# feiyeha/EGM-Unet

Measured on AMD Instinct MI355X. Metric: train images/sec at 3x512x512 bs=8/GPU, higher is better.
Workload: dtype bf16; 1 GPU; EGM-UNet GRFBUNet(3,2,base_c=32) fwd+5-term-loss+bwd+SGD, 8x3x512x512 per GPU (BASELINE.json configs[1]); global_batch=8, parallelism=dp1, launch=hipGraph replay, world_size=1

## Files before the change

### egm_unet_amd/csrc/common.h

```cpp
#pragma once
#include <hip/hip_runtime.h>
#include <stdint.h>
#include <stdio.h>
#include <stdlib.h>
#include <string.h>
#include <type_traits>
#include "../../include/egm_hip.h"

void egm_set_error(const char* fmt, ...);
#define EGM_FAIL(code, ...) do { egm_set_error(__VA_ARGS__); return (code); } while (0)
#define EGM_REQUIRE(cond, ...) do { if (!(cond)) EGM_FAIL(EGM_ERR_ARG, __VA_ARGS__); } while (0)
#define EGM_CHECK_LAUNCH(name) do { hipError_t e_ = hipGetLastError(); \
    if (e_ != hipSuccess) EGM_FAIL(EGM_ERR_LAUNCH, "%s: launch failed: %s", name, hipGetErrorString(e_)); } while (0)

static inline bool egm_aligned16(const void* p) { return (reinterpret_cast<uintptr_t>(p) & 15) == 0; }
static inline int egm_cdiv(long long a, long long b) { return (int)((a + b - 1) / b); }
static inline int egm_env_int(const char* name, int dflt) { const char* v = getenv(name); return v ? atoi(v) : dflt; }

template <auto Kernel> int egm_allow_max_lds(const char* what, int bytes = 160 * 1024) {
    static bool done = false;
    if (!done) {
        hipError_t e = hipFuncSetAttribute(reinterpret_cast<const void*>(Kernel), hipFuncAttributeMaxDynamicSharedMemorySize, bytes);
        if (e != hipSuccess) EGM_FAIL(EGM_ERR_LAUNCH, "%s: hipFuncSetAttribute: %s", what, hipGetErrorString(e));
        done = true;
// ... 28 lines not shown
__device__ __forceinline__ float bf16_to_f32(uint16_t b) { return __uint_as_float(((uint32_t)b) << 16); }
__device__ __forceinline__ uint16_t f32_to_bf16(float f) {
    __bf16 h = (__bf16)f;
    return *reinterpret_cast<uint16_t*>(&h);
}

template <typename T> struct TypeInfo;
template <> struct TypeInfo<float>  { static constexpr int kDtype = EGM_F32;  static constexpr int kVec = 4; };
template <> struct TypeInfo<bf16_t> { static constexpr int kDtype = EGM_BF16; static constexpr int kVec = 8; };

__device__ __forceinline__ float to_f32(float x) { return x; }
__device__ __forceinline__ float to_f32(bf16_t x) { return bf16_to_f32(x.v); }
template <typename T> __device__ __forceinline__ T from_f32(float x);
template <> __device__ __forceinline__ float from_f32<float>(float x) { return x; }
template <> __device__ __forceinline__ bf16_t from_f32<bf16_t>(float x) { bf16_t r; r.v = f32_to_bf16(x); return r; }

__device__ __forceinline__ void load8(const float* p, float (&v)[8]) {
    float4 a = *reinterpret_cast<const float4*>(p), b = *reinterpret_cast<const float4*>(p + 4);
    v[0] = a.x; v[1] = a.y; v[2] = a.z; v[3] = a.w; v[4] = b.x; v[5] = b.y; v[6] = b.z; v[7] = b.w;
}
#ifndef EGM_LOAD_MODE
#define EGM_LOAD_MODE 0
#endif
__device__ __forceinline__ void load8(const bf16_t* p, float (&v)[8]) {
#if EGM_LOAD_MODE == 2
    typedef __attribute__((ext_vector_type(4))) unsigned int u32x4_;
    const u32x4_ t = __builtin_nontemporal_load(reinterpret_cast<const u32x4_*>(p));
    uint4 a; a.x = t.x; a.y = t.y; a.z = t.z; a.w = t.w;
#else
    uint4 a = *reinterpret_cast<const uint4*>(p);
#endif
    v[0] = __uint_as_float(a.x << 16); v[1] = __uint_as_float(a.x & 0xffff0000u);
    v[2] = __uint_as_float(a.y << 16); v[3] = __uint_as_float(a.y & 0xffff0000u);
    v[4] = __uint_as_float(a.z << 16); v[5] = __uint_as_float(a.z & 0xffff0000u);
    v[6] = __uint_as_float(a.w << 16); v[7] = __uint_as_float(a.w & 0xffff0000u);
}
#ifndef EGM_STORE_MODE
#define EGM_STORE_MODE 2
#endif
#ifndef EGM_CONV_STORE_MODE
#define EGM_CONV_STORE_MODE 1
#endif
typedef __attribute__((ext_vector_type(4))) unsigned int egm_u32x4;
template <int MODE, typename V>
__device__ __forceinline__ void egm_store16_as(void* p, V a) {
    if (MODE == 1) asm volatile("global_store_dwordx4 %0, %1, off sc1\n\ts_nop 1" :: "v"(p), "v"(a) : "memory");
    else if (MODE == 2) __builtin_nontemporal_store(a, reinterpret_cast<V*>(p));
    else *reinterpret_cast<V*>(p) = a;
}
__device__ __forceinline__ void egm_store16_conv(void* p, uint4 v) {
    egm_u32x4 a; a.x = v.x; a.y = v.y; a.z = v.z; a.w = v.w;
    egm_store16_as<EGM_CONV_STORE_MODE>(p, a);
}
__device__ __forceinline__ void store8(float* p, const float (&v)[8]) {
    *reinterpret_cast<float4*>(p) = make_float4(v[0], v[1], v[2], v[3]);
    *reinterpret_cast<float4*>(p + 4) = make_float4(v[4], v[5], v[6], v[7]);
}
__device__ __forceinline__ void store8(bf16_t* p, const float (&v)[8]) {
// ... 122 lines not shown
```

### egm_unet_amd/csrc/pool_up.hip

```cpp
#include "common.h"

namespace {

template <typename T>
__global__ void nchw_to_nhwc_kernel(const float* __restrict__ src, T* __restrict__ dst, int ld, int N, int C, long long HW) {
    const long long total = (long long)N * HW;
    for (long long i = blockIdx.x * 256LL + threadIdx.x; i < total; i += (long long)gridDim.x * 256) {
        const long long n = i / HW, p = i - n * HW;
        for (int c0 = 0; c0 < ld; c0 += 8) {
            float v[8];
#pragma unroll
            for (int j = 0; j < 8; ++j) v[j] = (c0 + j < C) ? src[(n * C + c0 + j) * HW + p] : 0.f;
            store8(dst + i * ld + c0, v);
        }
    }
}
template <typename T>
__global__ void nhwc_to_nchw_kernel(const T* __restrict__ src, int ld, float* __restrict__ dst, int N, int C, long long HW) {
    const long long total = (long long)N * HW;
    for (long long i = blockIdx.x * 256LL + threadIdx.x; i < total; i += (long long)gridDim.x * 256) {
        const long long n = i / HW, p = i - n * HW;
        for (int c0 = 0; c0 < C; c0 += 8) {
            float v[8];
            load8(src + i * ld + c0, v);
// ... 56 lines not shown
                load8(add + off[k] * ldadd + cv * 8, a);
#pragma unroll
                for (int j = 0; j < 8; ++j) o[k][j] += a[j];
            }
        }
        store8(dx + base * lddx + cv * 8, o[0]);
        store8(dx + (base + 1) * lddx + cv * 8, o[1]);
        store8(dx + (base + W) * lddx + cv * 8, o[2]);
        store8(dx + (base + W + 1) * lddx + cv * 8, o[3]);
    }
}
template <typename T>
__global__ void zero_tail_kernel(T* __restrict__ dx, int lddx, int N, int H, int W, int C) {
    const int ncv = C >> 3;
    const long long total = (long long)N * H * W * ncv;
    float z[8]; zero8(z);
    for (long long i = blockIdx.x * 256LL + threadIdx.x; i < total; i += (long long)gridDim.x * 256) {
        long long p; int cv; egm_divmod(i, ncv, p, cv);
        int xx, yy; egm_pix_yx(p, H, W, yy, xx);
        if (yy >= (H & ~1) || xx >= (W & ~1)) store8(dx + p * lddx + cv * 8, z);
    }
}

struct Lerp { int i0, i1; float w0, w1; };
__device__ __forceinline__ Lerp lerp_coord(int dst, int in_size, int out_size) {
    const float scale = out_size > 1 ? (float)(in_size - 1) / (float)(out_size - 1) : 0.f;
    const float src = scale * (float)dst;
    Lerp l;
    l.i0 = (int)src;
    l.i1 = l.i0 + (l.i0 < in_size - 1 ? 1 : 0);
    l.w1 = src - (float)l.i0;
    l.w0 = 1.f - l.w1;
    return l;
}

template <typename T>
__global__ void upcat_fwd_kernel(const T* __restrict__ skip, int lds, const T* __restrict__ low, int ldl, T* __restrict__ out,
                                 int ldo, int N, int Hs, int Ws, int Cs, int Hl, int Wl, int Cl) {
    const int ncs = Cs >> 3, ncv = (Cs + Cl) >> 3, first = skip ? 0 : ncs, nw = ncv - first;
    const int Hu = 2 * Hl, Wu = 2 * Wl, py = (Hs - Hu) / 2, px = (Ws - Wu) / 2;
    const long long total = (long long)N * Hs * Ws * nw;
    for (long long i = blockIdx.x * 256LL + threadIdx.x; i < total; i += (long long)gridDim.x * 256) {
        const int cv = first + (int)(i % nw); const long long p = i / nw;
        float v[8];
        if (cv < ncs) {
            load8(skip + p * lds + cv * 8, v);
        } else {
            int x, y, n; egm_pix_nyx(p, Hs, Ws, n, y, x);
            const int uy = y - py, ux = x - px, c = (cv - ncs) * 8;
            zero8(v);
            if (uy >= 0 && uy < Hu && ux >= 0 && ux < Wu) {
                const Lerp ly = lerp_coord(uy, Hl, Hu), lx = lerp_coord(ux, Wl, Wu);
                const T* b = low + (long long)n * Hl * Wl * ldl + c;
                float a[8];
                load8(b + ((long long)ly.i0 * Wl + lx.i0) * ldl, a);
#pragma unroll
                for (int j = 0; j < 8; ++j) v[j] += ly.w0 * lx.w0 * a[j];
                load8(b + ((long long)ly.i0 * Wl + lx.i1) * ldl, a);
#pragma unroll
                for (int j = 0; j < 8; ++j) v[j] += ly.w0 * lx.w1 * a[j];
                load8(b + ((long long)ly.i1 * Wl + lx.i0) * ldl, a);
#pragma unroll
                for (int j = 0; j < 8; ++j) v[j] += ly.w1 * lx.w0 * a[j];
                load8(b + ((long long)ly.i1 * Wl + lx.i1) * ldl, a);
#pragma unroll
                for (int j = 0; j < 8; ++j) v[j] += ly.w1 * lx.w1 * a[j];
            }
        }
        store8(out + p * ldo + cv * 8, v);
    }
}

template <typename T>
__global__ void upcat_bwd_low_kernel(const T* __restrict__ dout, int ldo, T* __restrict__ dlow, int ldl, int N, int Hs, int Ws,
                                     int Cs, int Hl, int Wl, int Cl) {
// ... 610 lines not shown
```

### egm_unet_amd/egm_unet.py

```python
import math
from typing import Dict

import torch
import torch.nn as nn

from . import ops
from ._lib import ACT_NONE, ACT_RELU, ACT_SIGMOID
from .unet import DoubleConv, OutConv, Up, _SegNetBase


class StdPool(nn.Module):
    """Holder only (src/EGM-UNet.py:827-834); the statistics come from egm_mca_reduce."""


class MCAGate(nn.Module):
    def __init__(self, k_size, pool_types=("avg", "std")):
        super().__init__()
        self.pools = nn.ModuleList([nn.AdaptiveAvgPool2d(1) if p == "avg" else StdPool() for p in pool_types])
        self.conv = nn.Conv2d(1, 1, kernel_size=(1, k_size), stride=1, padding=(0, (k_size - 1) // 2), bias=False)
        self.sigmoid = nn.Sigmoid()
        self.weight = nn.Parameter(torch.rand(2))
        self.conv._egm_no_prepack = True


# ... 136 lines not shown
            BasicConv(in_channels, i, 3, padding=1),
            BasicConv(i, 2 * i, 3, stride=stride, padding=1, groups=2),
            BasicConv(2 * i, 2 * i, 3, padding=3 * visual, dilation=3 * visual, relu=False),
            BasicConv(2 * i, 2 * i, 1))
        self.concat_channels = in_channels + 6 * i
        self.fusion_conv = FusionConv(self.concat_channels, out_channels, factor=fusion_factor)
        self.shortcut = BasicConv(in_channels, out_channels, 1, stride, relu=False)
        self.relu = nn.ReLU(inplace=False)
        self.target_enhancer = nn.Sequential(nn.Conv2d(out_channels, 3, 3, padding=1), nn.Sigmoid())

    @staticmethod
    def _seq(seq, x, out):
        mods = list(seq)
        for m in mods[:-1]:
            x = m(x)
        return mods[-1](x, out=out)

    def cat_buffer(self, N, H, W, dtype, device):
        C, i2 = self.shortcut.conv.in_channels, 2 * self.inter_planes
        if i2 % 8 or C % 8:
            return None
        return ops.cat_slots(N, H, W, [C, i2, i2, i2], dtype, device)

    def forward(self, x, out=None, cat=None, pool=False):
        edge, x_e2, x_cat, x_sc = ops.fork_highpass3(x, 3)
        xe = self.edge_enhancer(None, x_e2, edge=edge)
        N, H, W, C = x.shape
        if cat is None:
            cat = self.cat_buffer(N, H, W, x.dtype, x.device) if C == self.shortcut.conv.in_channels else None
        if cat is not None:
            buf, (_, sd, se, sc) = cat
        else:
            buf, sd, se, sc = None, None, None, None
        bd, be, bc = self.branch_dir, self.branch_edge, self.branch_ctx
        xe_d, xe_e, xe_c = ops.fork(xe, 3)
        def item(m, t, o=None):
            return (t, m.conv, m.bn, ACT_RELU if m.relu is not None else ACT_NONE, m._dil, m._groups, o)

        d, e, c = ops.multi_conv_bn_act([item(bd[0], xe_d), item(be[0], xe_e), item(bc[0], xe_c)])
        e = be[1](e)
        e, c = ops.multi_conv_bn_act([item(be[2], e), item(bc[1], c)])
        d, e, c = ops.multi_conv_bn_act([item(bd[1], d), item(be[3], e), item(bc[2], c)])
        d, e, c = ops.multi_conv_bn_act([item(bd[2], d, sd), item(be[4], e, se), item(bc[3], c, sc)])
        cat = ops.cat_channels([x_cat, d, e, c], buf)
        out_f = self.fusion_conv(cat)
        sc = self.shortcut
        out_f = ops.conv_bn_ew(x_sc, sc.conv, sc.bn, ACT_NONE, out_f, ops.EW_SAR, alpha=self.scale)
        o_a, o_b = ops.fork(out_f, 2)
# ... 171 lines not shown
    def __init__(self, in_channels, out_channels, mid_channels=None, use_mca=True):
        if mid_channels is None:
            mid_channels = out_channels
        layers = [nn.Conv2d(in_channels, mid_channels, kernel_size=3, padding=1, bias=False), nn.BatchNorm2d(mid_channels), nn.ReLU(inplace=True)]
        if use_mca:
            layers.append(MCALayer(mid_channels))
        layers += [nn.Conv2d(mid_channels, out_channels, kernel_size=3, padding=1, bias=False), nn.BatchNorm2d(out_channels),
                   nn.ReLU(inplace=True), EdgeEnhancedGRFB(mid_channels, out_channels, stride=1, scale=0.1, visual=12)]
        super().__init__(*layers)
        self._mca = use_mca

    def forward(self, x, out=None, pool=False):
        o = 1 if self._mca else 0
        if self._mca:
            if ops.fuse_mca_bn():
                x = self[3](ops.conv_bn_lazy(x, self[0], self[1], ACT_RELU), exclusive=True)
            else:
                x = self[3](ops.conv_bn_act(x, self[0], self[1], ACT_RELU))
        else:
            x = ops.conv_bn_act(x, self[0], self[1], ACT_RELU)
        grfb = self[6 + o]
        N, H, W = x.shape[0], x.shape[1], x.shape[2]
        cat = grfb.cat_buffer(N, H, W, x.dtype, x.device) if self[3 + o].out_channels == grfb.shortcut.conv.in_channels else None
        x = ops.conv_bn_act(x, self[3 + o], self[4 + o], ACT_RELU, out=None if cat is None else cat[1][0])
        return grfb(x, out, cat, pool=pool)


class Down(nn.Sequential):
    def __init__(self, in_channels, out_channels, use_mca=True):
        super().__init__(nn.MaxPool2d(2, stride=2), DoubleConv1(in_channels, out_channels, use_mca=use_mca))

    def forward(self, x, out=None, pooled=None, pool=False):
        return self[1](ops.maxpool2(x) if pooled is None else pooled, out, pool=pool)


class GRFBUNet(_SegNetBase):
    def __init__(self, in_channels: int = 1, num_classes: int = 2, bilinear: bool = True, base_c: int = 64,
                 use_attention: bool = False, use_mca: bool = True):
        super().__init__()
        self.in_channels = in_channels
        self.num_classes = num_classes
        self.bilinear = bilinear
        self.in_conv = DoubleConv(in_channels, base_c)
        self.down1 = Down(base_c, base_c * 2, use_mca)
        self.down2 = Down(base_c * 2, base_c * 4, use_mca)
        self.down3 = Down(base_c * 4, base_c * 8, use_mca)
        factor = 2 if bilinear else 1
# ... 4 lines not shown
        self.up3 = Up(base_c * 4, base_c * 2 // factor, bilinear)
        self.up4 = Up(base_c * 2, base_c, bilinear)
        self.out_conv = OutConv(base_c, num_classes)

    def forward(self, x: torch.Tensor) -> Dict[str, torch.Tensor]:
        x = self._enter(x)
        bufs, slots = [None] * 4, [None] * 4
        if self.bilinear:
            N, H, W, _ = x.shape
            for k, up in enumerate((self.up4, self.up3, self.up2, self.up1)):
                cin = up.conv[0].in_channels
                cs = cin // 2
                h, w = H >> k, W >> k
                if cs % 8 == 0 and cin % 8 == 0 and (h << k) == H and (w << k) == W:
                    bufs[k], (slots[k], _) = ops.cat_slots(N, h, w, [cs, cin - cs], x.dtype, x.device)
        x1s, p1 = self.in_conv(x, slots[0], pool=True)
        x2s, p2 = self.down1(None, slots[1], pooled=p1, pool=True)
        x3s, p3 = self.down2(None, slots[2], pooled=p2, pool=True)
        x4s, p4 = self.down3(None, slots[3], pooled=p3, pool=True)
        d4 = self.down4(None, pooled=p4)
        if self.ddp_boundary is not None:
            self.ddp_boundary.extend([x1s, x2s, x3s, x4s, d4])
        x5 = self.attn1(d4)
        y = self.up1(x5, x4s, bufs[3])
        y = self.up2(y, x3s, bufs[2])
        y = self.up3(y, x2s, bufs[1])
        y = self.up4(y, x1s, bufs[0], lazy="force" if ops.fuse_cls() else False)
        return self._exit(self.out_conv(y, sole_consumer=True))
```

### egm_unet_amd/ops.py

```python
import ctypes
import os
import struct
import threading
import weakref
from collections import namedtuple

import torch
from torch.autograd import Function, Variable

from ._lib import ACT_NONE, ACT_RELU, ACT_SIGMOID, dtype_code, lib, ptr, stream


def pad8(c: int) -> int:
    return (c + 7) // 8 * 8


def _nhwc(t: torch.Tensor):
    assert t.dim() == 4, t.shape
    N, H, W, C = t.shape
    s = t.stride()
    ok = (s[3] == 1 and s[2] % 8 == 0 and s[2] >= C and s[1] == W * s[2] and s[0] == H * W * s[2]
          and t.data_ptr() % 16 == 0 and C % 8 == 0)
    if not ok:
        if C % 8:
# ... 1425 lines not shown
        (x,) = ctx.saved_tensors
        x, ldx = _nhwc(x)
        N, H, W, C = x.shape
        if gy is None:
            return gskip
        gy, ldg = _nhwc(gy)
        gx = torch.empty((N, H, W, C), dtype=x.dtype, device=x.device)
        dt = dtype_code(x.dtype)
        if gskip is None:
            lib().call("egm_maxpool2_bwd", dt, ptr(x), ldx, ptr(gy), ldg, ptr(gx), C, N, H, W, C, stream())
        elif (H | W) & 1:
            lib().call("egm_maxpool2_bwd", dt, ptr(x), ldx, ptr(gy), ldg, ptr(gx), C, N, H, W, C, stream())
            gx = _axpby(gx, 1.0, gskip, 1.0)
        else:
            gs, lds = _nhwc(gskip)
            lib().call("egm_maxpool2_bwd_add", dt, ptr(x), ldx, ptr(gy), ldg, ptr(gs), lds, ptr(gx), C, N, H, W, C, stream())
        return gx


def fork_maxpool2(x):
    return _ForkMaxPool2.apply(x)


class _UpCat(Function):

    @staticmethod
    def forward(ctx, skip, low, catbuf=None):
        skip, lds = _nhwc(skip)
        low, ldl = _nhwc(low)
        N, Hs, Ws, Cs = skip.shape
        _, Hl, Wl, Cl = low.shape
        inplace = False
        if catbuf is not None:
            cb = catbuf[0]
            inplace = (cb.is_contiguous() and tuple(cb.shape) == (N, Hs, Ws, Cs + Cl) and cb.dtype == skip.dtype
                       and cb.data_ptr() == skip.data_ptr() and lds == Cs + Cl)
        if inplace:
            out = cb
            lib().call("egm_upcat_fwd", dtype_code(skip.dtype), None, lds, ptr(low), ldl, ptr(out), Cs + Cl, N, Hs, Ws, Cs,
                       Hl, Wl, Cl, stream())
        else:
            out = torch.empty((N, Hs, Ws, Cs + Cl), dtype=skip.dtype, device=skip.device)
            lib().call("egm_upcat_fwd", dtype_code(skip.dtype), ptr(skip), lds, ptr(low), ldl, ptr(out), Cs + Cl, N, Hs, Ws, Cs,
                       Hl, Wl, Cl, stream())
        ctx.shape = (N, Hs, Ws, Cs, Hl, Wl, Cl)
        return out

    @staticmethod
    def backward(ctx, g):
        N, Hs, Ws, Cs, Hl, Wl, Cl = ctx.shape
        pend = _take_dz(g)
        gskip = glow = None
        if pend is not None:
            _, ga, gb = pend[1]
            if ctx.needs_input_grad[0]:
                gskip = ga
            if ctx.needs_input_grad[1]:
                glow = torch.empty((N, Hl, Wl, Cl), dtype=gb.dtype, device=gb.device)
                lib().call("egm_upcat_bwd_low", dtype_code(gb.dtype), ptr(gb), Cl, ptr(glow), Cl, N, Hs, Ws, 0, Hl, Wl, Cl, stream())
            return gskip, glow, None
        g, ldo = _nhwc(g)
        if ctx.needs_input_grad[0]:
            gskip = g[..., :Cs]
        if ctx.needs_input_grad[1]:
            glow = torch.empty((N, Hl, Wl, Cl), dtype=g.dtype, device=g.device)
            lib().call("egm_upcat_bwd_low", dtype_code(g.dtype), ptr(g), ldo, ptr(glow), Cl, N, Hs, Ws, Cs, Hl, Wl, Cl, stream())
        return gskip, glow, None


def upcat(skip, low, catbuf=None):
    out = _UpCat.apply(skip, low, None if catbuf is None else [catbuf])
    out._egm_split = skip.shape[3]
    return out


class _Fork2(Function):

    @staticmethod
    def forward(ctx, x):
        return x.view_as(x), x.view_as(x)

    @staticmethod
    def backward(ctx, ga, gb):
        if ga is None:
            return gb
        if gb is None:
            return ga
        ga, lda = _nhwc(ga)
        gb, ldb = _nhwc(gb)
        out = torch.empty(ga.shape, dtype=ga.dtype, device=ga.device)
        lib().call("egm_axpby", dtype_code(ga.dtype), ptr(ga), lda, 1.0, ptr(gb), ldb, 1.0, ptr(out), out.shape[3], _npix(ga),
                   ga.shape[3], stream())
        return out

# ... 116 lines not shown

class _Highpass3(Function):
    @staticmethod
    def forward(ctx, x):
        return _hp(x)

    @staticmethod
    def backward(ctx, g):
        return _hp(g)


def highpass3(x):
    return _Highpass3.apply(x)


class _ForkHighpass(Function):

    @staticmethod
    def forward(ctx, x, n):
        return (_hp(x),) + tuple(x.view_as(x) for _ in range(n))

    @staticmethod
    def backward(ctx, ghp, *gs):
        gs = [g for g in gs if g is not None]
        if ghp is None:
            return (_Fork.backward(ctx, *gs)[0] if gs else None), None
        if not gs:
            return _hp(ghp), None
        while len(gs) > 3:
            gs = gs[:2] + [_Fork.backward(ctx, *gs[2:])[0]]
        a, lda = _nhwc(ghp)
        N, H, W, C = a.shape
        ts = [_nhwc(t) for t in gs] + [(None, 0)] * (3 - len(gs))
        out = torch.empty(a.shape, dtype=a.dtype, device=a.device)
        lib().call("egm_sum4_hp", dtype_code(a.dtype), ptr(a), lda, ptr(ts[0][0]), ts[0][1], ptr(ts[1][0]), ts[1][1], ptr(ts[2][0]), ts[2][1],
                   ptr(out), C, N, H, W, C, stream())
        return out, None


def fork_highpass3(x, n):
    return _ForkHighpass.apply(x, n)


class _GateMul(Function):
    @staticmethod
    def forward(ctx, x, w):
        x, ldx = _nhwc(x)
        w, ldw = _nhwc(w)
        out = torch.empty(x.shape, dtype=x.dtype, device=x.device)
        lib().call("egm_gate_mul_fwd", dtype_code(x.dtype), ptr(x), ldx, ptr(w), ldw, ptr(out), x.shape[3], _npix(x), x.shape[3], stream())
        ctx.save_for_backward(x, w)
        return out

    @staticmethod
    def backward(ctx, g):
        x, w = ctx.saved_tensors
        x, ldx = _nhwc(x); w, ldw = _nhwc(w); g, ldg = _nhwc(g)
        C = x.shape[3]
        dx = torch.empty(x.shape, dtype=x.dtype, device=x.device)
        dw = torch.empty(x.shape, dtype=x.dtype, device=x.device)
        lib().call("egm_gate_mul_bwd", dtype_code(x.dtype), ptr(g), ldg, ptr(x), ldx, ptr(w), ldw, ptr(dx), C, ptr(dw), C, _npix(x), C, stream())
        return dx, dw

# ... 747 lines not shown
```

### egm_unet_amd/unet.py

```python
from typing import Dict

import torch
import torch.nn as nn

from . import ops
from ._lib import ACT_RELU, require_gpu


class DoubleConv(nn.Sequential):

    def __init__(self, in_channels, out_channels, mid_channels=None, use_attention=False):
        if mid_channels is None:
            mid_channels = out_channels
        super().__init__(
            nn.Conv2d(in_channels, mid_channels, kernel_size=3, padding=1, bias=False),
            nn.BatchNorm2d(mid_channels),
            nn.ReLU(inplace=True),
            nn.Conv2d(mid_channels, out_channels, kernel_size=3, padding=1, bias=False),
            nn.BatchNorm2d(out_channels),
            nn.ReLU(inplace=True),
        )

    def forward(self, x, out=None, lazy=False, pool=False):
        x = ops.conv_bn_act(x, self[0], self[1], ACT_RELU)
# ... 8 lines not shown

    def __init__(self, in_channels, out_channels):
        super().__init__(nn.MaxPool2d(2, stride=2), DoubleConv(in_channels, out_channels))

    def forward(self, x, pooled=None, pool=False):
        return self[1](ops.maxpool2(x) if pooled is None else pooled, pool=pool)


class Up(nn.Module):

    def __init__(self, in_channels, out_channels, bilinear=True, use_attention=False):
        super().__init__()
        self.bilinear = bilinear
        if bilinear:
            self.up = nn.Upsample(scale_factor=2, mode="bilinear", align_corners=True)
            self.conv = DoubleConv(in_channels, out_channels, in_channels // 2)
        else:
            self.up = nn.ConvTranspose2d(in_channels, in_channels // 2, kernel_size=2, stride=2)
            self.conv = DoubleConv(in_channels, out_channels)

    def forward(self, x1, x2, catbuf=None, lazy=False):
        if self.bilinear:
            return self.conv(ops.upcat(x2, x1, catbuf), lazy=lazy)
        x1 = ops.conv_transpose2x2(x1, self.up, (x2.shape[1], x2.shape[2]))
        return self.conv(ops.cat_channels([x2, x1]), lazy=lazy)


class OutConv(nn.Sequential):

    def __init__(self, in_channels, num_classes):
        super().__init__(nn.Conv2d(in_channels, num_classes, kernel_size=1))

    def forward(self, x, sole_consumer=False):
        if sole_consumer and ops.bn_act_cls_ok(x, self[0].weight):
            out = ops.bn_act_cls(x, self[0].weight, self[0].bias)
            out._egm_nchw_logits = True
            return out
        was_lazy = isinstance(x, ops.Lazy)
        return ops.conv2d(ops.materialize(x), self[0].weight, self[0].bias, defer_dgrad=sole_consumer and not was_lazy)


class _SegNetBase(nn.Module):

    compute_dtype = torch.float32
    ddp_boundary = None

    def set_compute_dtype(self, dtype):
# ... 37 lines not shown
        self.in_conv = DoubleConv(in_channels, base_c)
        self.down1 = Down(base_c, base_c * 2)
        self.down2 = Down(base_c * 2, base_c * 4)
        self.down3 = Down(base_c * 4, base_c * 8)
        factor = 2 if bilinear else 1
        self.down4 = Down(base_c * 8, base_c * 16 // factor)
        self.up1 = Up(base_c * 16, base_c * 8 // factor, bilinear)
        self.up2 = Up(base_c * 8, base_c * 4 // factor, bilinear)
        self.up3 = Up(base_c * 4, base_c * 2 // factor, bilinear)
        self.up4 = Up(base_c * 2, base_c, bilinear)
        self.out_conv = OutConv(base_c, num_classes)

    def forward(self, x: torch.Tensor) -> Dict[str, torch.Tensor]:
        x = self._enter(x)
        x1s, p1 = self.in_conv(x, pool=True)
        x2s, p2 = self.down1(None, pooled=p1, pool=True)
        x3s, p3 = self.down2(None, pooled=p2, pool=True)
        x4s, p4 = self.down3(None, pooled=p3, pool=True)
        x5 = self.down4(None, pooled=p4)
        if self.ddp_boundary is not None:
            x5, x5d = ops.fork2(x5)
            self.ddp_boundary.extend([x1s, x2s, x3s, x4s, x5d])
            x5 = x5d
        y = self.up1(x5, x4s)
        y = self.up2(y, x3s)
        y = self.up3(y, x2s)
        y = self.up4(y, x1s, lazy="force" if ops.fuse_cls() else False)
        return self._exit(self.out_conv(y, sole_consumer=True))
```

### include/egm_hip.h

```cpp
#ifndef EGM_HIP_H
#define EGM_HIP_H

#ifdef __cplusplus
extern "C" {
#endif

typedef void* egm_stream_t;

enum egm_status { EGM_OK = 0, EGM_ERR_ARG = -1, EGM_ERR_LAUNCH = -2, EGM_ERR_UNSUPPORTED = -3 };
enum egm_dtype { EGM_F32 = 0, EGM_BF16 = 1 };
enum egm_act { EGM_ACT_NONE = 0, EGM_ACT_RELU = 1, EGM_ACT_SIGMOID = 2, EGM_ACT_SILU = 3  };

int egm_version(void);
const char* egm_last_error(void);
int egm_device_ok(void);

int egm_nchw_to_nhwc(int dtype, const void* src_f32, void* dst, int ld, int N, int C, int H, int W, egm_stream_t s);
int egm_nhwc_to_nchw(int dtype, const void* src, int ld, void* dst_f32, int N, int C, int H, int W, egm_stream_t s);

int egm_conv_pack(int dtype, const void* w_oihw_f32, void* wf, void* wd, int Cout, int Cin, int KH, int KW, int groups,
                  egm_stream_t s);
int egm_conv_pack_chunk(void);
int egm_conv_pack_multi(int dtype, const void* table_dev, int n, long long total_chunks, egm_stream_t s);
int egm_group_begin(void);
// ... 113 lines not shown
int egm_conv1x1_bwd_slabs(long long npix);
int egm_conv1x1_bwd(int dtype, const egm_conv1x1_bwd_desc* descs, int n, egm_stream_t s);

int egm_maxpool2_fwd(int dtype, const void* x, int ldx, void* y, int ldy, int N, int H, int W, int C, egm_stream_t s);
int egm_maxpool2_bwd(int dtype, const void* x, int ldx, const void* dy, int lddy, void* dx, int lddx, int N, int H, int W,
                     int C, egm_stream_t s);
int egm_maxpool2_bwd_add(int dtype, const void* x, int ldx, const void* dy, int lddy, const void* add, int ldadd, void* dx, int lddx,
                         int N, int H, int W, int C, egm_stream_t s);
int egm_bn_act_fwd_pool(int dtype, const void* y, int ldy, const float* scale, const float* shift, int act, void* z, int ldz,
                        void* pooled, int ldp, int N, int H, int W, int C, egm_stream_t s);
int egm_bn_pool_bwd_blocks(int N, int H, int W, int C);
int egm_bn_pool_bwd_reduce(int dtype, const void* gskip, int ldgs, const void* gpool, int ldgp, const void* y, int ldy,
                           const float* scale, const float* shift, const float* save_mean, const float* save_rstd, int act,
                           float* partials, int N, int H, int W, int C, egm_stream_t s);
int egm_bn_pool_bwd_apply(int dtype, const void* gskip, int ldgs, const void* gpool, int ldgp, const void* y, int ldy,
                          const float* scale, const float* shift, const float* save_mean, const float* save_rstd, int act, int train,
                          const float* sums, void* dy, int lddy, int N, int H, int W, int C, egm_stream_t s);
int egm_gate3_fwd_pool(int dtype, const void* x, int ldx, const void* t, int ldt, void* out, int ldo, void* pooled, int ldp, int N,
                       int H, int W, int C, egm_stream_t s);
int egm_gate3_pool_bwd(int dtype, const void* gskip, int ldgs, const void* gpool, int ldgp, const void* x, int ldx, const void* t,
                       int ldt, void* dx, int lddx, void* dt, int lddt, int N, int H, int W, int C, egm_stream_t s);
int egm_upcat_fwd(int dtype, const void* skip, int lds, const void* low, int ldl, void* out, int ldo, int N, int Hs, int Ws,
                  int Cs, int Hl, int Wl, int Cl, egm_stream_t s);
int egm_upcat_bwd_low(int dtype, const void* dout, int ldo, void* dlow, int ldl, int N, int Hs, int Ws, int Cs, int Hl,
                      int Wl, int Cl, egm_stream_t s);

int egm_axpby(int dtype, const void* a, int lda, float alpha, const void* b, int ldb, float beta, void* out, int ldo,
              long long npix, int C, egm_stream_t s);
int egm_sum4(int dtype, const void* a, int lda, const void* b, int ldb, const void* c, int ldc, const void* d, int ldd, void* out,
             int ldo, long long npix, int C, egm_stream_t s);
int egm_sum4_hp(int dtype, const void* a, int lda, const void* b, int ldb, const void* c, int ldc, const void* d, int ldd, void* out,
                int ldo, int N, int H, int W, int C, egm_stream_t s);
int egm_vec_add_f32(float* y, const float* x, long long n, egm_stream_t s);
int egm_fill_f32(float* y, float v, long long n, egm_stream_t s);
int egm_copy_cols_f32(const float* src, int ld_src, int col0_src, float* dst, int ld_dst, int col0_dst, int rows, int ncols,
                      egm_stream_t s);

int egm_highpass3(int dtype, const void* x, int ldx, void* out, int ldo, int N, int H, int W, int C, egm_stream_t s);
int egm_gate_mul_fwd(int dtype, const void* x, int ldx, const void* w, int ldw, void* out, int ldo, long long npix, int C,
                     egm_stream_t s);
int egm_gate_mul_bwd(int dtype, const void* g, int ldg, const void* x, int ldx, const void* w, int ldw, void* dx, int lddx,
                     void* dw, int lddw, long long npix, int C, egm_stream_t s);

int egm_scale_add_relu_fwd(int dtype, const void* a, int lda, float alpha, const void* b, int ldb, void* out, int ldo,
                           long long npix, int C, egm_stream_t s);
int egm_scale_add_relu_bwd(int dtype, const void* g, int ldg, const void* out, int ldo, float alpha, void* da, int ldda,
// ... 362 lines not shown
```

Measured before the change: 697.3 images/s.

## Fuse BN+ReLU into high-pass fork and bilinear upsample-concat forward kernels

```diff
diff --git a/egm_unet_amd/csrc/bn_stencil_fused.hip b/egm_unet_amd/csrc/bn_stencil_fused.hip
--- /dev/null
+++ b/egm_unet_amd/csrc/bn_stencil_fused.hip
@@ -0,0 +1,214 @@
+#include "bn_elem.h"
+#include "lerp.h"
+
+namespace {
+
+__device__ __forceinline__ void load_coef8(const float* __restrict__ scale, const float* __restrict__ shift, int c, bool ok, float (&sc)[8],
+                                           float (&sh)[8]) {
+#pragma unroll
+    for (int j = 0; j < 8; ++j) { sc[j] = ok ? scale[c + j] : 0.f; sh[j] = ok ? shift[c + j] : 0.f; }
+}
+
+constexpr int HP_TY = 8, HP_TX = 16, HP_CB = 32;
+__global__ __launch_bounds__(256) void bn_act_hp_fwd_kernel(const bf16_t* __restrict__ y, int ldy, const float* __restrict__ scale,
+                                                            const float* __restrict__ shift, int act, bf16_t* __restrict__ z, int ldz,
+                                                            bf16_t* __restrict__ edge, int lde, int N, int H, int W, int C, int tiles_x,
+                                                            int tiles_y, int nchunk) {
+    constexpr int TY = HP_TY, TX = HP_TX, NB = 3;
+    constexpr int PY = TY + 2, PX = TX + 2, NST = PY * PX * 4, NS = (NST + 255) / 256;
+    __shared__ __attribute__((aligned(16))) bf16_t sz[PY * PX * HP_CB];
+    const int tid = threadIdx.x, vt = tid & 3;
+    int b = xcd_contiguous_item(blockIdx.x, gridDim.x);
+    const int chunk = b % nchunk; b /= nchunk;
+    const int tx = b % tiles_x; b /= tiles_x;
+    const int ty = b % tiles_y; const int n = b / tiles_y;
+    const int y0 = ty * TY, x0 = tx * TX, c0 = chunk * HP_CB;
+    const int nvec = (C - c0 < HP_CB ? C - c0 : HP_CB) >> 3;
+    const bool okv = vt < nvec;
+    const int c = c0 + vt * 8;
+    const long long img = (long long)n * H * W;
+    float sc[8], sh[8];
+    load_coef8(scale, shift, c, okv, sc, sh);
+    static_assert(NS == NB, "one batch");
+#pragma unroll
+    for (int k0 = 0; k0 < NS; k0 += NB) {
+        uint4 raw[NB];
+#pragma unroll
+        for (int kk = 0; kk < NB; ++kk) {
+            const int i = tid + (k0 + kk) * 256, pix = i >> 2, ry = pix / PX, rx = pix - ry * PX;
+            const int gy = y0 + ry - 1, gx = x0 + rx - 1;
+            raw[kk] = make_uint4(0, 0, 0, 0);
+            if (i < NST && okv && gy >= 0 && gy < H && gx >= 0 && gx < W)
+                raw[kk] = *reinterpret_cast<const uint4*>(y + (img + (long long)gy * W + gx) * ldy + c);
+        }
+#pragma unroll
+        for (int kk = 0; kk < NB; ++kk) {
+            const int i = tid + (k0 + kk) * 256, pix = i >> 2, ry = pix / PX, rx = pix - ry * PX;
+            const int gy = y0 + ry - 1, gx = x0 + rx - 1;
+            if (i >= NST) break;
+            bf16_t* dst = sz + pix * HP_CB + vt * 8;
+            if (okv && gy >= 0 && gy < H && gx >= 0 && gx < W) {
+                float a[8];
+                load8(raw[kk], a);
+#pragma unroll
+                for (int j = 0; j < 8; ++j) a[j] = bn_fwd_elem<true>(a[j], sc[j], sh[j], act);
+                store8_lds(dst, a);
+                if (ry >= 1 && ry <= TY && rx >= 1 && rx <= TX)
+                    store8(z + (img + (long long)gy * W + gx) * ldz + c, a);
+            } else {
+                *reinterpret_cast<uint4*>(dst) = make_uint4(0, 0, 0, 0);
+            }
+        }
+    }
+    __syncthreads();
+    for (int i = tid; i < TY * TX * 4; i += 256) {
+        const int pix = i >> 2, ly = pix / TX, lx = pix - ly * TX;
+        const int yy = y0 + ly, xx = x0 + lx;
+        if (!okv || yy >= H || xx >= W) continue;
+        const bf16_t* base = sz + ((ly + 1) * PX + lx + 1) * HP_CB + vt * 8;
+        float s[8], cc[8], v[8];
+        zero8(s);
+        load8(base, cc);
+#pragma unroll
+        for (int r = -1; r <= 1; ++r)
+#pragma unroll
+            for (int q = -1; q <= 1; ++q) {
+                if (yy + r < 0 || yy + r >= H || xx + q < 0 || xx + q >= W) continue;
+                load8(base + (r * PX + q) * HP_CB, v);
+#pragma unroll
+                for (int j = 0; j < 8; ++j) s[j] += v[j];
+            }
+#pragma unroll
+        for (int j = 0; j < 8; ++j) cc[j] -= s[j] * (1.f / 9.f);
+        store8(edge + (img + (long long)yy * W + xx) * lde + c, cc);
+    }
+}
+
+constexpr int UF_TY = 16, UF_TX = 32, UF_CB = 32, UF_LR = UF_TY / 2 + 3, UF_LC = UF_TX / 2 + 3;
+__global__ __launch_bounds__(256) void bn_act_upcat_fwd_kernel(const bf16_t* __restrict__ skip, int lds, const bf16_t* __restrict__ low, int ldl,
+                                                               const float* __restrict__ scale, const float* __restrict__ shift, int act,
+                                                               bf16_t* __restrict__ out, int ldo, int N, int Hs, int Ws, int Cs, int Hl, int Wl,
+                                                               int Cl, int tiles_x, int tiles_y, int nsc, int nlc) {
+    __shared__ __attribute__((aligned(16))) bf16_t sl[UF_LR * UF_LC * UF_CB];
+    __shared__ Lerp sly[UF_TY], slx[UF_TX];
+    const int tid = threadIdx.x, vt = tid & 3;
+    int b = xcd_contiguous_item(blockIdx.x, gridDim.x);
+    const int nchunk = nsc + nlc;
+    const int chunk = b % nchunk; b /= nchunk;
+    const int tx = b % tiles_x; b /= tiles_x;
+    const int ty = b % tiles_y; const int n = b / tiles_y;
+    const int y0 = ty * UF_TY, x0 = tx * UF_TX;
+    const long long img = (long long)n * Hs * Ws;
+    if (chunk < nsc) {
+        const int c0 = chunk * UF_CB, nvec = (Cs - c0 < UF_CB ? Cs - c0 : UF_CB) >> 3;
+        for (int i = tid; i < UF_TY * UF_TX * 4; i += 256) {
+            const int pix = i >> 2, ly = pix / UF_TX, lx = pix - ly * UF_TX;
+            const int yy = y0 + ly, xx = x0 + lx;
+            if (vt >= nvec || yy >= Hs || xx >= Ws) continue;
+            const long long p = img + (long long)yy * Ws + xx;
+            float v[8];
+            load8(skip + p * lds + c0 + vt * 8, v);
+            store8(out + p * ldo + c0 + vt * 8, v);
+        }
+        return;
+    }
+    const int c0 = (chunk - nsc) * UF_CB, nvec = (Cl - c0 < UF_CB ? Cl - c0 : UF_CB) >> 3;
+    const bool okv = vt < nvec;
+    const int c = c0 + vt * 8;
+    const int Hu = 2 * Hl, Wu = 2 * Wl, py = (Hs - Hu) / 2, px = (Ws - Wu) / 2;
+    const int yend = y0 + UF_TY < Hs ? y0 + UF_TY : Hs, xend = x0 + UF_TX < Ws ? x0 + UF_TX : Ws;
+    const int uy_lo = y0 - py > 0 ? y0 - py : 0, uy_hi = yend - 1 - py < Hu - 1 ? yend - 1 - py : Hu - 1;
+    const int ux_lo = x0 - px > 0 ? x0 - px : 0, ux_hi = xend - 1 - px < Wu - 1 ? xend - 1 - px : Wu - 1;
+    const bool any = uy_lo <= uy_hi && ux_lo <= ux_hi;
+    int r0 = 0, nr = 0, q0 = 0, nq = 0;
+    if (any) {
+        r0 = lerp_coord<true>(uy_lo, Hl, Hu).i0; nr = lerp_coord<true>(uy_hi, Hl, Hu).i1 - r0 + 1;
+        q0 = lerp_coord<true>(ux_lo, Wl, Wu).i0; nq = lerp_coord<true>(ux_hi, Wl, Wu).i1 - q0 + 1;
+    }
+    if (tid < UF_TY) {
+        const int uy = y0 + tid - py;
+        Lerp l; l.i0 = 0; l.i1 = 0; l.w0 = 0.f; l.w1 = 0.f;
+        if (uy >= uy_lo && uy <= uy_hi) { l = lerp_coord<true>(uy, Hl, Hu); l.i0 -= r0; l.i1 -= r0; }
+        sly[tid] = l;
+    } else if (tid >= 64 && tid < 64 + UF_TX) {
+        const int ux = x0 + tid - 64 - px;
+        Lerp l; l.i0 = 0; l.i1 = 0; l.w0 = 0.f; l.w1 = 0.f;
+        if (ux >= ux_lo && ux <= ux_hi) { l = lerp_coord<true>(ux, Wl, Wu); l.i0 -= q0; l.i1 -= q0; }
+        slx[tid - 64] = l;
+    }
+    float sc[8], sh[8];
+    load_coef8(scale, shift, c, okv, sc, sh);
+    const bf16_t* __restrict__ lowb = low + (long long)n * Hl * Wl * ldl + c;
+    for (int i = tid; i < nr * nq * 4; i += 256) {
+        const int pix = i >> 2, rr = pix / nq, qq = pix - rr * nq;
+        if (!okv) continue;
+        float a[8];
+        load8(lowb + ((long long)(r0 + rr) * Wl + q0 + qq) * ldl, a);
+#pragma unroll
+        for (int j = 0; j < 8; ++j) a[j] = bn_fwd_elem<true>(a[j], sc[j], sh[j], act);
+        store8_lds(sl + (rr * UF_LC + qq) * UF_CB + vt * 8, a);
+    }
+    __syncthreads();
+    for (int i = tid; i < UF_TY * UF_TX * 4; i += 256) {
+        const int pix = i >> 2, ly = pix / UF_TX, lx = pix - ly * UF_TX;
+        const int yy = y0 + ly, xx = x0 + lx;
+        if (!okv || yy >= Hs || xx >= Ws) continue;
+        const int uy = yy - py, ux = xx - px;
+        float v[8];
+        zero8(v);
+        if (uy >= 0 && uy < Hu && ux >= 0 && ux < Wu) {
+            const Lerp ay = sly[ly], ax = slx[lx];
+            const bf16_t* sb = sl + vt * 8;
+            float a[8];
+            load8(sb + (ay.i0 * UF_LC + ax.i0) * UF_CB, a);
+#pragma unroll
+            for (int j = 0; j < 8; ++j) v[j] += ay.w0 * ax.w0 * a[j];
+            load8(sb + (ay.i0 * UF_LC + ax.i1) * UF_CB, a);
+#pragma unroll
+            for (int j = 0; j < 8; ++j) v[j] += ay.w0 * ax.w1 * a[j];
+            load8(sb + (ay.i1 * UF_LC + ax.i0) * UF_CB, a);
+#pragma unroll
+            for (int j = 0; j < 8; ++j) v[j] += ay.w1 * ax.w0 * a[j];
+            load8(sb + (ay.i1 * UF_LC + ax.i1) * UF_CB, a);
+#pragma unroll
+            for (int j = 0; j < 8; ++j) v[j] += ay.w1 * ax.w1 * a[j];
+        }
+        store8(out + (img + (long long)yy * Ws + xx) * ldo + Cs + c, v);
+    }
+}
+
+}
+
+extern "C" int egm_bn_act_hp_fwd(int dtype, const void* y, int ldy, const float* scale, const float* shift, int act, void* z, int ldz,
+                                 void* edge, int lde, int N, int H, int W, int C, egm_stream_t s) {
+    EGM_REQUIRE(dtype == EGM_BF16, "bn_act_hp_fwd: bf16 only (dtype %d); other types take egm_bn_act_fwd + egm_highpass3", dtype);
+    EGM_REQ_VEC("bn_act_hp_fwd", y, ldy, C); EGM_REQ_VEC("bn_act_hp_fwd", z, ldz, C); EGM_REQ_VEC("bn_act_hp_fwd", edge, lde, C);
+    EGM_REQUIRE(scale && shift && N > 0 && H > 0 && W > 0 && act >= EGM_ACT_NONE && act <= EGM_ACT_SILU, "bn_act_hp_fwd: bad args");
+    const int nchunk = egm_cdiv(C, HP_CB);
+    const int tiles_y = egm_cdiv(H, HP_TY), tiles_x = egm_cdiv(W, HP_TX);
+    const long long grid = (long long)N * tiles_y * tiles_x * nchunk;
+    EGM_REQUIRE(grid < (1ll << 31), "bn_act_hp_fwd: tensor too large");
+    hipLaunchKernelGGL(bn_act_hp_fwd_kernel, dim3((unsigned)grid), dim3(256), 0, (hipStream_t)s, (const bf16_t*)y, ldy, scale, shift, act,
+                       (bf16_t*)z, ldz, (bf16_t*)edge, lde, N, H, W, C, tiles_x, tiles_y, nchunk);
+    EGM_CHECK_LAUNCH("bn_act_hp_fwd");
+    return EGM_OK;
+}
+
+extern "C" int egm_bn_act_upcat_fwd(int dtype, const void* skip, int lds, const void* low, int ldl, const float* scale, const float* shift,
+                                    int act, void* out, int ldo, int N, int Hs, int Ws, int Cs, int Hl, int Wl, int Cl, egm_stream_t s) {
+    EGM_REQUIRE(dtype == EGM_BF16, "bn_act_upcat_fwd: bf16 only (dtype %d); other types take egm_bn_act_fwd + egm_upcat_fwd", dtype);
+    if (skip != nullptr) EGM_REQ_VEC("bn_act_upcat_fwd", skip, lds, Cs);
+    EGM_REQUIRE(Cs > 0 && Cs % 8 == 0, "bn_act_upcat_fwd: bad Cs %d", Cs);
+    EGM_REQ_VEC("bn_act_upcat_fwd", low, ldl, Cl);
+    EGM_REQ_VEC("bn_act_upcat_fwd", out, ldo, Cs + Cl);
+    EGM_REQUIRE(scale && shift && act >= EGM_ACT_NONE && act <= EGM_ACT_SILU, "bn_act_upcat_fwd: bad args");
+    EGM_REQUIRE(N > 0 && Hl > 0 && Wl > 0 && Hs >= 2 * Hl && Ws >= 2 * Wl, "bn_act_upcat_fwd: skip must be at least 2x the low-res size");
+    const int tiles_y = egm_cdiv(Hs, UF_TY), tiles_x = egm_cdiv(Ws, UF_TX);
+    const int nsc = skip ? egm_cdiv(Cs, UF_CB) : 0, nlc = egm_cdiv(Cl, UF_CB);
+    const long long grid = (long long)N * tiles_y * tiles_x * (nsc + nlc);
+    EGM_REQUIRE(grid < (1ll << 31), "bn_act_upcat_fwd: tensor too large");
+    hipLaunchKernelGGL(bn_act_upcat_fwd_kernel, dim3((unsigned)grid), dim3(256), 0, (hipStream_t)s, (const bf16_t*)skip, lds, (const bf16_t*)low,
+                       ldl, scale, shift, act, (bf16_t*)out, ldo, N, Hs, Ws, Cs, Hl, Wl, Cl, tiles_x, tiles_y, nsc, nlc);
+    EGM_CHECK_LAUNCH("bn_act_upcat_fwd");
+    return EGM_OK;
+}
diff --git a/egm_unet_amd/csrc/common.h b/egm_unet_amd/csrc/common.h
--- a/egm_unet_amd/csrc/common.h
+++ b/egm_unet_amd/csrc/common.h
@@ -74,6 +74,12 @@
 #ifndef EGM_LOAD_MODE
 #define EGM_LOAD_MODE 0
 #endif
+__device__ __forceinline__ void load8(uint4 a, float (&v)[8]) {
+    v[0] = __uint_as_float(a.x << 16); v[1] = __uint_as_float(a.x & 0xffff0000u);
+    v[2] = __uint_as_float(a.y << 16); v[3] = __uint_as_float(a.y & 0xffff0000u);
+    v[4] = __uint_as_float(a.z << 16); v[5] = __uint_as_float(a.z & 0xffff0000u);
+    v[6] = __uint_as_float(a.w << 16); v[7] = __uint_as_float(a.w & 0xffff0000u);
+}
 __device__ __forceinline__ void load8(const bf16_t* p, float (&v)[8]) {
 #if EGM_LOAD_MODE == 2
     typedef __attribute__((ext_vector_type(4))) unsigned int u32x4_;
@@ -82,10 +88,7 @@
 #else
     uint4 a = *reinterpret_cast<const uint4*>(p);
 #endif
-    v[0] = __uint_as_float(a.x << 16); v[1] = __uint_as_float(a.x & 0xffff0000u);
-    v[2] = __uint_as_float(a.y << 16); v[3] = __uint_as_float(a.y & 0xffff0000u);
-    v[4] = __uint_as_float(a.z << 16); v[5] = __uint_as_float(a.z & 0xffff0000u);
-    v[6] = __uint_as_float(a.w << 16); v[7] = __uint_as_float(a.w & 0xffff0000u);
+    load8(a, v);
 }
 #ifndef EGM_STORE_MODE
 #define EGM_STORE_MODE 2
diff --git a/egm_unet_amd/csrc/lerp.h b/egm_unet_amd/csrc/lerp.h
--- /dev/null
+++ b/egm_unet_amd/csrc/lerp.h
@@ -0,0 +1,19 @@
+#pragma once
+#include "common.h"
+
+struct Lerp { int i0, i1; float w0, w1; };
+__device__ __forceinline__ float egm_mul_rounded(float a, float b) {
+#pragma clang fp contract(off)
+    return a * b;
+}
+template <bool ROUNDED = false>
+__device__ __forceinline__ Lerp lerp_coord(int dst, int in_size, int out_size) {
+    const float scale = out_size > 1 ? (float)(in_size - 1) / (float)(out_size - 1) : 0.f;
+    const float src = ROUNDED ? egm_mul_rounded(scale, (float)dst) : scale * (float)dst;
+    Lerp l;
+    l.i0 = (int)src;
+    l.i1 = l.i0 + (l.i0 < in_size - 1 ? 1 : 0);
+    l.w1 = src - (float)l.i0;
+    l.w0 = 1.f - l.w1;
+    return l;
+}
diff --git a/egm_unet_amd/csrc/pool_up.hip b/egm_unet_amd/csrc/pool_up.hip
--- a/egm_unet_amd/csrc/pool_up.hip
+++ b/egm_unet_amd/csrc/pool_up.hip
@@ -1,4 +1,5 @@
 #include "common.h"
+#include "lerp.h"
 
 namespace {
 
@@ -102,18 +103,6 @@
     }
 }
 
-struct Lerp { int i0, i1; float w0, w1; };
-__device__ __forceinline__ Lerp lerp_coord(int dst, int in_size, int out_size) {
-    const float scale = out_size > 1 ? (float)(in_size - 1) / (float)(out_size - 1) : 0.f;
-    const float src = scale * (float)dst;
-    Lerp l;
-    l.i0 = (int)src;
-    l.i1 = l.i0 + (l.i0 < in_size - 1 ? 1 : 0);
-    l.w1 = src - (float)l.i0;
-    l.w0 = 1.f - l.w1;
-    return l;
-}
-
 template <typename T>
 __global__ void upcat_fwd_kernel(const T* __restrict__ skip, int lds, const T* __restrict__ low, int ldl, T* __restrict__ out,
                                  int ldo, int N, int Hs, int Ws, int Cs, int Hl, int Wl, int Cl) {
@@ -130,7 +119,7 @@
             const int uy = y - py, ux = x - px, c = (cv - ncs) * 8;
             zero8(v);
             if (uy >= 0 && uy < Hu && ux >= 0 && ux < Wu) {
-                const Lerp ly = lerp_coord(uy, Hl, Hu), lx = lerp_coord(ux, Wl, Wu);
+                const Lerp ly = lerp_coord<true>(uy, Hl, Hu), lx = lerp_coord<true>(ux, Wl, Wu);
                 const T* b = low + (long long)n * Hl * Wl * ldl + c;
                 float a[8];
                 load8(b + ((long long)ly.i0 * Wl + lx.i0) * ldl, a);
diff --git a/egm_unet_amd/egm_unet.py b/egm_unet_amd/egm_unet.py
--- a/egm_unet_amd/egm_unet.py
+++ b/egm_unet_amd/egm_unet.py
@@ -182,8 +182,8 @@
             return None
         return ops.cat_slots(N, H, W, [C, i2, i2, i2], dtype, device)
 
-    def forward(self, x, out=None, cat=None, pool=False):
-        edge, x_e2, x_cat, x_sc = ops.fork_highpass3(x, 3)
+    def forward(self, x, out=None, cat=None, pool=False, x_slot=None):
+        edge, x_e2, x_cat, x_sc = ops.fork_highpass3(x, 3, out=x_slot)
         xe = self.edge_enhancer(None, x_e2, edge=edge)
         N, H, W, C = x.shape
         if cat is None:
@@ -401,7 +401,10 @@
         grfb = self[6 + o]
         N, H, W = x.shape[0], x.shape[1], x.shape[2]
         cat = grfb.cat_buffer(N, H, W, x.dtype, x.device) if self[3 + o].out_channels == grfb.shortcut.conv.in_channels else None
-        x = ops.conv_bn_act(x, self[3 + o], self[4 + o], ACT_RELU, out=None if cat is None else cat[1][0])
+        slot = None if cat is None else cat[1][0]
+        if ops.bn_hp_fusable(x.dtype):
+            return grfb(ops.conv_bn_act(x, self[3 + o], self[4 + o], ACT_RELU, lazy="force"), out, cat, pool=pool, x_slot=slot)
+        x = ops.conv_bn_act(x, self[3 + o], self[4 + o], ACT_RELU, out=slot)
         return grfb(x, out, cat, pool=pool)
 
 
@@ -452,8 +455,9 @@
         if self.ddp_boundary is not None:
             self.ddp_boundary.extend([x1s, x2s, x3s, x4s, d4])
         x5 = self.attn1(d4)
-        y = self.up1(x5, x4s, bufs[3])
-        y = self.up2(y, x3s, bufs[2])
-        y = self.up3(y, x2s, bufs[1])
+        lazy_up = "force" if self.bilinear and ops.bn_up_fusable(x5.dtype) else False
+        y = self.up1(x5, x4s, bufs[3], lazy=lazy_up)
+        y = self.up2(y, x3s, bufs[2], lazy=lazy_up)
+        y = self.up3(y, x2s, bufs[1], lazy=lazy_up)
         y = self.up4(y, x1s, bufs[0], lazy="force" if ops.fuse_cls() else False)
         return self._exit(self.out_conv(y, sole_consumer=True))
diff --git a/egm_unet_amd/ops.py b/egm_unet_amd/ops.py
--- a/egm_unet_amd/ops.py
+++ b/egm_unet_amd/ops.py
@@ -1471,54 +1471,91 @@
     return _ForkMaxPool2.apply(x)
 
 
+fuse_bn_up = _Switch("EGM_FUSE_BN_UP", "1",
+                     """Get / set whether the bilinear upsample of an Up block applies the BatchNorm+ReLU of the Up block in front itself
+                     (bf16; egm_bn_act_upcat_fwd), so that block's low-resolution output is never written (tests compare both ways).""")
+
+
+def _upcat_forward(ctx, skip, low, catbuf, low_bn=None):
+    skip, lds = _nhwc(skip)
+    low, ldl = _nhwc(low)
+    N, Hs, Ws, Cs = skip.shape
+    _, Hl, Wl, Cl = low.shape
+    inplace = False
+    if catbuf is not None:
+        cb = catbuf[0]
+        inplace = (cb.is_contiguous() and tuple(cb.shape) == (N, Hs, Ws, Cs + Cl) and cb.dtype == skip.dtype
+                   and cb.data_ptr() == skip.data_ptr() and lds == Cs + Cl)
+    out = cb if inplace else torch.empty((N, Hs, Ws, Cs + Cl), dtype=skip.dtype, device=skip.device)
+    src = None if inplace else ptr(skip)
+    if low_bn is None:
+        lib().call("egm_upcat_fwd", dtype_code(skip.dtype), src, lds, ptr(low), ldl, ptr(out), Cs + Cl, N, Hs, Ws, Cs, Hl, Wl, Cl, stream())
+    else:
+        coef, act = low_bn
+        lib().call("egm_bn_act_upcat_fwd", dtype_code(skip.dtype), src, lds, ptr(low), ldl, ptr(coef[0]), ptr(coef[1]), act, ptr(out), Cs + Cl,
+                   N, Hs, Ws, Cs, Hl, Wl, Cl, stream())
+    ctx.shape = (N, Hs, Ws, Cs, Hl, Wl, Cl)
+    return out
+
+
+def _upcat_backward(ctx, g):
+    N, Hs, Ws, Cs, Hl, Wl, Cl = ctx.shape
+    pend = _take_dz(g)
+    gskip = glow = None
+    if pend is not None:
+        _, ga, gb = pend[1]
+        if ctx.needs_input_grad[0]:
+            gskip = ga
+        if ctx.needs_input_grad[1]:
+            glow = torch.empty((N, Hl, Wl, Cl), dtype=gb.dtype, device=gb.device)
+            lib().call("egm_upcat_bwd_low", dtype_code(gb.dtype), ptr(gb), Cl, ptr(glow), Cl, N, Hs, Ws, 0, Hl, Wl, Cl, stream())
+        return gskip, glow
+    g, ldo = _nhwc(g)
+    if ctx.needs_input_grad[0]:
+        gskip = g[..., :Cs]
+    if ctx.needs_input_grad[1]:
+        glow = torch.empty((N, Hl, Wl, Cl), dtype=g.dtype, device=g.device)
+        lib().call("egm_upcat_bwd_low", dtype_code(g.dtype), ptr(g), ldo, ptr(glow), Cl, N, Hs, Ws, Cs, Hl, Wl, Cl, stream())
+    return gskip, glow
+
+
 class _UpCat(Function):
 
     @staticmethod
     def forward(ctx, skip, low, catbuf=None):
-        skip, lds = _nhwc(skip)
-        low, ldl = _nhwc(low)
-        N, Hs, Ws, Cs = skip.shape
-        _, Hl, Wl, Cl = low.shape
-        inplace = False
-        if catbuf is not None:
-            cb = catbuf[0]
-            inplace = (cb.is_contiguous() and tuple(cb.shape) == (N, Hs, Ws, Cs + Cl) and cb.dtype == skip.dtype
-                       and cb.data_ptr() == skip.data_ptr() and lds == Cs + Cl)
-        if inplace:
-            out = cb
-            lib().call("egm_upcat_fwd", dtype_code(skip.dtype), None, lds, ptr(low), ldl, ptr(out), Cs + Cl, N, Hs, Ws, Cs,
-                       Hl, Wl, Cl, stream())
-        else:
-            out = torch.empty((N, Hs, Ws, Cs + Cl), dtype=skip.dtype, device=skip.device)
-            lib().call("egm_upcat_fwd", dtype_code(skip.dtype), ptr(skip), lds, ptr(low), ldl, ptr(out), Cs + Cl, N, Hs, Ws, Cs,
-                       Hl, Wl, Cl, stream())
-        ctx.shape = (N, Hs, Ws, Cs, Hl, Wl, Cl)
-        return out
-
-    @staticmethod
-    def backward(ctx, g):
-        N, Hs, Ws, Cs, Hl, Wl, Cl = ctx.shape
-        pend = _take_dz(g)
-        gskip = glow = None
-        if pend is not None:
-            _, ga, gb = pend[1]
-            if ctx.needs_input_grad[0]:
-                gskip = ga
-            if ctx.needs_input_grad[1]:
-                glow = torch.empty((N, Hl, Wl, Cl), dtype=gb.dtype, device=gb.device)
-                lib().call("egm_upcat_bwd_low", dtype_code(gb.dtype), ptr(gb), Cl, ptr(glow), Cl, N, Hs, Ws, 0, Hl, Wl, Cl, stream())
-            return gskip, glow, None
-        g, ldo = _nhwc(g)
-        if ctx.needs_input_grad[0]:
-            gskip = g[..., :Cs]
-        if ctx.needs_input_grad[1]:
-            glow = torch.empty((N, Hl, Wl, Cl), dtype=g.dtype, device=g.device)
-            lib().call("egm_upcat_bwd_low", dtype_code(g.dtype), ptr(g), ldo, ptr(glow), Cl, N, Hs, Ws, Cs, Hl, Wl, Cl, stream())
-        return gskip, glow, None
+        return _upcat_forward(ctx, skip, low, catbuf)
+
+    @staticmethod
+    def backward(ctx, g):
+        return _upcat_backward(ctx, g) + (None,)
+
+
+class _UpCatBn(Function):
+
+    @staticmethod
+    def forward(ctx, skip, y, coef, act, catbuf=None):
+        return _upcat_forward(ctx, skip, y, catbuf, (coef, act))
+
+    @staticmethod
+    def backward(ctx, g):
+        return _upcat_backward(ctx, g) + (None, None, None)
+
+
+def _bn_up_ok(dtype):
+    return fuse_bn_up.on and dtype == torch.bfloat16
+
+
+def bn_up_fusable(dtype):
+    return _bn_up_ok(dtype) and _fold_packs() is None
 
 
 def upcat(skip, low, catbuf=None):
-    out = _UpCat.apply(skip, low, None if catbuf is None else [catbuf])
+    if isinstance(low, Lazy) and not (_bn_up_ok(low.dtype) and skip.dtype == low.dtype):
+        low = low.materialize()
+    if isinstance(low, Lazy):
+        out = _UpCatBn.apply(skip, low.y, low.coef, low.act, None if catbuf is None else [catbuf])
+    else:
+        out = _UpCat.apply(skip, low, None if catbuf is None else [catbuf])
     out._egm_split = skip.shape[3]
     return out
 
@@ -1681,23 +1718,63 @@
 
     @staticmethod
     def backward(ctx, ghp, *gs):
-        gs = [g for g in gs if g is not None]
-        if ghp is None:
-            return (_Fork.backward(ctx, *gs)[0] if gs else None), None
-        if not gs:
-            return _hp(ghp), None
-        while len(gs) > 3:
-            gs = gs[:2] + [_Fork.backward(ctx, *gs[2:])[0]]
-        a, lda = _nhwc(ghp)
-        N, H, W, C = a.shape
-        ts = [_nhwc(t) for t in gs] + [(None, 0)] * (3 - len(gs))
-        out = torch.empty(a.shape, dtype=a.dtype, device=a.device)
-        lib().call("egm_sum4_hp", dtype_code(a.dtype), ptr(a), lda, ptr(ts[0][0]), ts[0][1], ptr(ts[1][0]), ts[1][1], ptr(ts[2][0]), ts[2][1],
-                   ptr(out), C, N, H, W, C, stream())
-        return out, None
-
-
-def fork_highpass3(x, n):
+        return _fork_highpass_backward(ctx, ghp, gs), None
+
+
+def _fork_highpass_backward(ctx, ghp, gs):
+    gs = [g for g in gs if g is not None]
+    if ghp is None:
+        return _Fork.backward(ctx, *gs)[0] if gs else None
+    if not gs:
+        return _hp(ghp)
+    while len(gs) > 3:
+        gs = gs[:2] + [_Fork.backward(ctx, *gs[2:])[0]]
+    a, lda = _nhwc(ghp)
+    N, H, W, C = a.shape
+    ts = [_nhwc(t) for t in gs] + [(None, 0)] * (3 - len(gs))
+    out = torch.empty(a.shape, dtype=a.dtype, device=a.device)
+    lib().call("egm_sum4_hp", dtype_code(a.dtype), ptr(a), lda, ptr(ts[0][0]), ts[0][1], ptr(ts[1][0]), ts[1][1], ptr(ts[2][0]), ts[2][1],
+               ptr(out), C, N, H, W, C, stream())
+    return out
+
+
+fuse_bn_hp = _Switch("EGM_FUSE_BN_HP", "1",
+                     """Get / set whether the EdgeEnhancedGRFB's entry high-pass applies the BatchNorm+ReLU of the DoubleConv1 conv in front
+                     itself (bf16; egm_bn_act_hp_fwd): the tensor is written and its edge map formed in one pass (tests compare both ways).""")
+
+
+class _ForkHighpassBn(Function):
+
+    @staticmethod
+    def forward(ctx, y, coef, act, n, out_slot):
+        y, ldy = _nhwc(y)
+        N, H, W, C = y.shape
+        z, ldz = _slot_or_new(out_slot, (N, H, W, C), y.dtype, y.device)
+        edge = torch.empty((N, H, W, C), dtype=y.dtype, device=y.device)
+        lib().call("egm_bn_act_hp_fwd", dtype_code(y.dtype), ptr(y), ldy, ptr(coef[0]), ptr(coef[1]), act, ptr(z), ldz, ptr(edge), C,
+                   N, H, W, C, stream())
+        return (edge,) + tuple(z.view_as(z) for _ in range(n))
+
+    @staticmethod
+    def backward(ctx, ghp, *gs):
+        return _fork_highpass_backward(ctx, ghp, gs), None, None, None, None
+
+
+def _bn_hp_ok(dtype):
+    return fuse_bn_hp.on and dtype == torch.bfloat16
+
+
+def bn_hp_fusable(dtype):
+    return _bn_hp_ok(dtype) and _fold_packs() is None
+
+
+def fork_highpass3(x, n, out=None):
+    if isinstance(x, Lazy):
+        if _bn_hp_ok(x.dtype):
+            return _ForkHighpassBn.apply(x.y, x.coef, x.act, n, None if out is None else [out])
+        x = x.materialize(out)
+    elif out is not None:
+        x = materialize(x, out)
     return _ForkHighpass.apply(x, n)
 
 
diff --git a/egm_unet_amd/unet.py b/egm_unet_amd/unet.py
--- a/egm_unet_amd/unet.py
+++ b/egm_unet_amd/unet.py
@@ -54,7 +54,7 @@
     def forward(self, x1, x2, catbuf=None, lazy=False):
         if self.bilinear:
             return self.conv(ops.upcat(x2, x1, catbuf), lazy=lazy)
-        x1 = ops.conv_transpose2x2(x1, self.up, (x2.shape[1], x2.shape[2]))
+        x1 = ops.conv_transpose2x2(ops.materialize(x1), self.up, (x2.shape[1], x2.shape[2]))
         return self.conv(ops.cat_channels([x2, x1]), lazy=lazy)
 
 
@@ -138,8 +138,9 @@
             x5, x5d = ops.fork2(x5)
             self.ddp_boundary.extend([x1s, x2s, x3s, x4s, x5d])
             x5 = x5d
-        y = self.up1(x5, x4s)
-        y = self.up2(y, x3s)
-        y = self.up3(y, x2s)
+        lazy_up = "force" if self.bilinear and ops.bn_up_fusable(x5.dtype) else False
+        y = self.up1(x5, x4s, lazy=lazy_up)
+        y = self.up2(y, x3s, lazy=lazy_up)
+        y = self.up3(y, x2s, lazy=lazy_up)
         y = self.up4(y, x1s, lazy="force" if ops.fuse_cls() else False)
         return self._exit(self.out_conv(y, sole_consumer=True))
diff --git a/include/egm_hip.h b/include/egm_hip.h
--- a/include/egm_hip.h
+++ b/include/egm_hip.h
@@ -159,6 +159,10 @@
                        int ldt, void* dx, int lddx, void* dt, int lddt, int N, int H, int W, int C, egm_stream_t s);
 int egm_upcat_fwd(int dtype, const void* skip, int lds, const void* low, int ldl, void* out, int ldo, int N, int Hs, int Ws,
                   int Cs, int Hl, int Wl, int Cl, egm_stream_t s);
+int egm_bn_act_hp_fwd(int dtype, const void* y, int ldy, const float* scale, const float* shift, int act, void* z, int ldz,
+                      void* edge, int lde, int N, int H, int W, int C, egm_stream_t s);
+int egm_bn_act_upcat_fwd(int dtype, const void* skip, int lds, const void* low, int ldl, const float* scale, const float* shift,
+                         int act, void* out, int ldo, int N, int Hs, int Ws, int Cs, int Hl, int Wl, int Cl, egm_stream_t s);
 int egm_upcat_bwd_low(int dtype, const void* dout, int ldo, void* dlow, int ldl, int N, int Hs, int Ws, int Cs, int Hl,
                       int Wl, int Cl, egm_stream_t s);
 
```

New measurement: 706.8 images/s, median of 6. 1.4% higher.
